# omnirevolve/omnirevolve-image-processor

Hardware: AMD Instinct MI355X
Metric: Mpx/s end-to-end (color->order) (higher is better)
Workload: dtype u8/i32 raster + f32/f64 geometry; 1 GPU; 4096x4096 BGR image, 8 colour layers, stages 02->12 (k-means fit, masks, edges, contours, scale, sort, intra dedup, cross dedup, plot order), default A4 canvas 8400x11880; parallelism=one GPU, one pipeline per colour layer, ops_last_step_rank0=4261, exchange=none

## Files before the change

omnirevolve-image-processor_amd/csrc/raster04.hip:

```cpp
#include "bitplane.h"
#include "walker.h"
#include <rocprim/rocprim.hpp>
#include <algorithm>
#include <cstdlib>

__global__ __launch_bounds__(256) void k_gather_head_layers(const unsigned* __restrict__ keys, const unsigned* __restrict__ cs, unsigned nc, unsigned* __restrict__ out) {
    unsigned i = blockIdx.x * 256 + threadIdx.x;
    if (i < nc) out[i] = keys[cs[i]] >> 26;
}

__global__ __launch_bounds__(64) void k_trace(WalkArgs A) {
    unsigned i = blockIdx.x;
    if (i >= A.nc) return;
    trace_component(A, A.comp_order ? A.comp_order[i] : i);
}
__global__ __launch_bounds__(64) void k_write_walks(WalkArgs A, int layer, const unsigned* __restrict__ kept_slots, const unsigned long long* __restrict__ kept_off, unsigned n_kept,
                                                    unsigned long long total, unsigned chunk) {
    for (unsigned long long ci = blockIdx.x; ci * chunk < total; ci += gridDim.x) {
        const unsigned long long p0 = ci * chunk, p1 = p0 + chunk < total ? p0 + chunk : total;
        write_chunk(A, layer, kept_slots, kept_off, n_kept, p0, p1);
    }
}
__global__ void k_totals_flag(const int* __restrict__ over, unsigned* __restrict__ pad_of_total) { *pad_of_total = (unsigned)*over; }
struct WSum {
// ... 337 lines not shown
    layer_first[K] = NC;
    for (int l = 0; l < K; l++) A.total_fg[l] = (long long)R.h_cs[layer_first[l + 1]] - (long long)R.h_cs[layer_first[l]];
    {
        unsigned long long *kin, *kout; unsigned *idin, *idout;
        { Carve L; L.each(NC, kin, kout, idin, idout); HIPC(c, L.commit(LN(c).vtmp[VT0_ORDER_SORT], 64)); }
        hipLaunchKernelGGL(k_comp_order_keys, dim3(cdiv(NC, 256)), block, 0, LN(c).stream, keys, comp_start, NC, kin, idin);
        HIPC(c, orip_with_tmp(c, [&](void* tmp, size_t& bytes) { return rocprim::radix_sort_pairs(tmp, bytes, kin, kout, idin, idout, (size_t)NC, 0, 40, LN(c).stream); }));
        R.order = LN(c).vtmp[VT0_ORDER].as<unsigned>();
        HIPC(c, hipMemcpyAsync(LN(c).vtmp[VT0_ORDER].p, idout, (size_t)NC * 4, hipMemcpyDeviceToDevice, LN(c).stream));
    }
    HIPC(c, LN(c).vtmp[VT0_WINFO].ensure((size_t)2 * M * sizeof(WalkInfo) + 64));
    A.memo = LN(c).vtmp[VT0_MEMO].as<unsigned>(); A.winfo = LN(c).vtmp[VT0_WINFO].as<WalkInfo>();
    HIPC(c, LN(c).vtmp[VT0_LOG_USED].ensure((size_t)(NC + 1) * 4 + 64));
    A.log_used = LN(c).vtmp[VT0_LOG_USED].as<unsigned>();
    HIPC(c, hipStreamSynchronize(LN(c).stream));
    R.ready = true;
    if (!getenv("ORIP_TRACE_LATE"))
        for (int l = 0; l < R.K; l++) {
            if (R.layer_first[l] == R.layer_first[l + 1]) continue;
            LaneGuard g(c, l + 1);
            if (!g.ok) continue;
            HIPC(c, orip_pf08_drain(c));
            ORIP_TRY(trace_launch(c, R, l, trace_log_f0()));
        }
    return 0;
}

static int trace_launch(orip_ctx* c, Prep04& R, int layer, unsigned F) {
    const unsigned c0 = R.layer_first[layer], c1 = R.layer_first[layer + 1];
    const unsigned b0 = R.h_cs[c0], b1 = R.h_cs[c1];
    const unsigned Ml = b1 - b0, NCl = c1 - c0;
    const size_t plane = (size_t)R.A.plane;
    if ((uint64_t)F * R.M + (uint64_t)256 * R.NC + 64 >= 0xffffffffull) ORIP_FAIL(c, "skeleton too large for the walk logs (factor %u)", F);
    const size_t nlog = (size_t)F * Ml + (size_t)64 * NCl + 8, nstep = (size_t)F * Ml + (size_t)256 * NCl + 8;
    WalkStore& WS = c->wstore[layer];
    WS.epoch++; WS.n = 0;
    HIPC(c, WS.log.ensure(nlog * 16 + 64));
    HIPC(c, LN(c).vtmp[VTL_STEPLOG].ensure(nstep + 64));
    WalkArgs A = R.A;
    A.logbuf = WS.log.as<unsigned>() - 4 * ((size_t)F * b0 + (size_t)64 * c0);
    A.steplog = LN(c).vtmp[VTL_STEPLOG].as<u8>() - ((size_t)F * b0 + (size_t)256 * c0);
    A.cap_factor = F; A.comp_order = R.order + c0; A.nc = NCl;
    int* d_over = &LN(c).flags.as<LaneFlags>()->trace_overflow; A.overflow = d_over;
    if (R.chains) HIPC(c, hipStreamWaitEvent(LN(c).stream, c->ln[0].ev3, 0));
    if (R.F[layer])
        hipLaunchKernelGGL(k_clear_visited_layer, dim3(cdiv(Ml, 256)), dim3(256), 0, LN(c).stream, A.st + plane * layer, A.lin + b0, (int64_t)Ml);
    hipLaunchKernelGGL(k_clear_memo_layer, dim3(cdiv((int64_t)2 * Ml, 256)), dim3(256), 0, LN(c).stream, reinterpret_cast<uint4*>(A.memo + plane * 8 * layer), A.lin + b0, (int64_t)2 * Ml);
    HIPC(c, hipMemsetAsync(A.winfo + 2 * (size_t)b0, 0, (size_t)2 * Ml * sizeof(WalkInfo), LN(c).stream));
    HIPC(c, hipMemsetAsync(d_over, 0, 4, LN(c).stream));
    if (getenv("ORIP_WALK_DBG")) {
        HIPC(c, LN(c).vtmp[VT_LEAVES].ensure((size_t)NCl * 256 + 64)); HIPC(c, hipMemsetAsync(LN(c).vtmp[VT_LEAVES].p, 0, (size_t)NCl * 256, LN(c).stream));
        A.dbg = LN(c).vtmp[VT_LEAVES].as<unsigned long long>() - 32ull * c0;
    }
    { ProfScope ps(c, "k_trace"); hipLaunchKernelGGL(k_trace, dim3(NCl), dim3(64), 0, LN(c).stream, A); }
    HIPC(c, hipGetLastError());
    R.F[layer] = F; R.launched[layer] = true;
    return 0;
}
static int trace_finish(orip_ctx* c, Prep04& R, int layer) {
    const unsigned c0 = R.layer_first[layer], c1 = R.layer_first[layer + 1];
    const unsigned b0 = R.h_cs[c0], b1 = R.h_cs[c1];
    const unsigned Ml = b1 - b0;
    dim3 block(256);
    int* d_over = &LN(c).flags.as<LaneFlags>()->trace_overflow;
    const unsigned nslots = 2u * Ml, sl0 = 2u * b0;
    const size_t ns1 = (size_t)nslots + 1;
    WSum *ws, *wo; { Carve L; L.each(ns1, ws, wo); HIPC(c, L.commit(LN(c).vtmp[VTL_CAPS], 256)); }
    WalkStore& WS = c->wstore[layer];
    WSum h_tot; unsigned log_shift = 0; WalkArgs A;
    for (;;) {
    log_shift = (unsigned)((size_t)R.F[layer] * b0 + (size_t)64 * c0);
    A = R.A;
    A.logbuf = WS.log.as<unsigned>() - 4 * (size_t)log_shift;
    A.steplog = LN(c).vtmp[VTL_STEPLOG].as<u8>() - ((size_t)R.F[layer] * b0 + (size_t)256 * c0);
    A.cap_factor = R.F[layer]; A.overflow = d_over;
    hipLaunchKernelGGL(k_winfo_lens, dim3(cdiv(nslots + 1, 256)), block, 0, LN(c).stream, A, sl0, nslots, ws);
    { WSum zero; zero.pts = 0; zero.paths = zero.own = zero.pieces = zero.pad = 0; HIPC(c, orip_with_tmp(c, [&](void* tmp, size_t& bytes) { return rocprim::exclusive_scan(tmp, bytes, ws, wo, zero, ns1, rocprim::plus<WSum>(), LN(c).stream); })); }
    hipLaunchKernelGGL(k_totals_flag, dim3(1), dim3(1), 0, LN(c).stream, d_over, &wo[nslots].pad);
    HIPC(c, hipMemcpyAsync(&h_tot, wo + nslots, sizeof(WSum), hipMemcpyDeviceToHost, LN(c).stream));
    {
        const unsigned NCl = c1 - c0;
        WS.ent_cap = (int64_t)8 * Ml + 64;
        HIPC(c, WS.lxy.ensure(((size_t)R.F[layer] * Ml + (size_t)64 * NCl + 8) * 8 + 64));
        HIPC(c, WS.ent_idx.ensure((size_t)WS.ent_cap * 4 + 64));
        HIPC(c, WS.cnt.ensure(64));
        HIPC(c, hipMemsetAsync(WS.cnt.p, 0, 4, LN(c).stream));
        hipLaunchKernelGGL(k_ent_fill, dim3(NCl, 8), block, 0, LN(c).stream, A, c0, log_shift, WS.lxy.as<int2>(), WS.ent_idx.as<unsigned>(), WS.cnt.as<unsigned>(), (unsigned)WS.ent_cap);
    }
    HIPC(c, hipStreamSynchronize(LN(c).stream));
    if (!h_tot.pad) break;
    if (h_tot.pad == 2) ORIP_FAIL(c, "internal error: the walker of layer %d stopped making progress", layer);
    ORIP_TRY(trace_launch(c, R, layer, R.F[layer] * 4));
    }
    if (getenv("ORIP_WALK_DBG")) {
        const unsigned NCl = c1 - c0;
        std::vector<unsigned long long> h((size_t)NCl * 32);
        HIPC(c, hipMemcpy(h.data(), LN(c).vtmp[VT_LEAVES].p, h.size() * 8, hipMemcpyDeviceToHost));
        unsigned long long tot[32] = {0}; size_t big = 0;
        for (size_t i = 0; i < h.size(); i++) tot[i % 32] += h[i];
        for (size_t i = 0; i < NCl; i++) if (h[i * 32 + 7] > h[big * 32 + 7]) big = i;
        const unsigned long long* d = &h[big * 32];
        fprintf(stderr, "[walk dbg] layer %d NC=%u M=%u F=%u: w1=%llu s1=%llu w2=%llu s2=%llu hit=%llu det=%llu tiles=%llu | largest fg=%llu: w1=%llu s1=%llu w2=%llu s2=%llu hit=%llu det=%llu tiles=%llu jumped=%llu calls=%llu rounds=%llu\n",
                layer, NCl, Ml, R.F[layer], tot[0], tot[1], tot[2], tot[3], tot[4], tot[5], tot[6], d[7], d[0], d[1], d[2], d[3], d[4], d[5], d[6], d[15], d[22], d[23]);
        if (d[8]) fprintf(stderr, "[walk prof] layer %d largest component: cycles total=%llu window loads=%llu scans=%llu look-ups=%llu | look-ups=%llu loop exits=%llu\n",
                          layer, d[8], d[9], d[10], d[11], d[12], d[13]);
        if (d[8]) fprintf(stderr, "[walk prof]   inside the look-ups: duplicate check %llu cycles (exact check in %llu look-ups); forced stretches %llu cycles in %llu calls, %llu rounds; stepping loop %llu cycles; walk start + end %llu cycles\n", d[14], d[20], d[16], d[17], d[18], d[19], d[21]);
    }
    const unsigned long long h_pts = h_tot.pts; const unsigned h_paths = h_tot.paths, h_own = h_tot.own, h_pieces = h_tot.pieces;
    DPolys& P = c->polys[ORIP_SLOT_CONTOURS][layer];
    P.total = (int64_t)h_pts; P.n = (int64_t)h_paths;
    P.virt = true; P.pts_ok = false; P.vident = true; P.vlayer = layer; P.vepoch = WS.epoch; P.scaled = false;
    HIPC(c, P.off.ensure((size_t)(P.n + 1) * 8 + 64));
    HIPC(c, WS.walk.ensure((size_t)std::max(h_paths, 1u) * sizeof(VWalk) + 64));
    HIPC(c, WS.piece.ensure((size_t)std::max(h_pieces, 1u) * sizeof(VPiece) + 64));
    HIPC(c, WS.own.ensure((size_t)std::max(h_own, 1u) * 8 + 64));
    HIPC(c, LN(c).vtmp[VTL_CELLS].ensure((size_t)std::max(h_paths, 1u) * 4 + 64));
    unsigned* kept_slots = LN(c).vtmp[VTL_CELLS].as<unsigned>();
    WS.n = P.n; WS.W = R.A.W; WS.n_own = h_own;
    hipLaunchKernelGGL(k_vwalk_fill, dim3(cdiv(nslots + 1, 256)), block, 0, LN(c).stream, A, sl0, nslots, wo, log_shift,
                       WS.walk.as<VWalk>(), WS.piece.as<VPiece>(), kept_slots, P.off.as<int64_t>());
    if (h_paths) {
        ProfScope ps(c, "k_write_walks");
        const unsigned chunk = 2048;
        hipLaunchKernelGGL(k_vown, dim3((unsigned)std::min<unsigned long long>(((unsigned long long)h_own + chunk - 1) / chunk, 262144ull)), dim3(64), 0, LN(c).stream, A, kept_slots, WS.walk.as<VWalk>(), h_paths,
                           WS.own.as<int2>(), h_own, chunk);
    }
    HIPC(c, hipGetLastError());
    R.launched[layer] = false;
    return 0;
}

int orip_contours_layer_impl(orip_ctx* c, int layer, bool sync) {
    Prep04* R = static_cast<Prep04*>(c->prep04);
    if (!R || !R->ready) ORIP_FAIL(c, "orip_contours_prepare has not run");
    if (layer < 0 || layer >= R->K) ORIP_FAIL(c, "bad layer %d (prepared for %d layers)", layer, R->K);
    if (R->M == 0 || R->layer_first[layer] == R->layer_first[layer + 1]) return 0;
    ORIP_LANE(c, layer + 1);
    if (!R->launched[layer]) ORIP_TRY(trace_launch(c, *R, layer, trace_log_f0()));
    ORIP_TRY(trace_finish(c, *R, layer));
    if (sync) HIPC(c, hipStreamSynchronize(LN(c).stream));
    return 0;
}
extern "C" int orip_contours_layer(orip_ctx* c, int layer) {
    orip_enter(c);
    return orip_contours_layer_impl(c, layer, true);
}

extern "C" int orip_find_contours(orip_ctx* c) {
    orip_enter(c);
    ORIP_TRY(orip_contours_prepare(c));
    Prep04& R = *static_cast<Prep04*>(c->prep04);
    if (R.M == 0) return 0;
    for (int l = 0; l < R.K; l++) if (R.layer_first[l] != R.layer_first[l + 1] && !R.launched[l]) { ORIP_LANE(c, l + 1); ORIP_TRY(trace_launch(c, R, l, trace_log_f0())); }
    for (int l = 0; l < R.K; l++) if (R.launched[l]) { ORIP_LANE(c, l + 1); ORIP_TRY(trace_finish(c, R, l)); HIPC(c, hipStreamSynchronize(LN(c).stream)); }
    return 0;
}
// ... 10 lines not shown
```

omnirevolve-image-processor_amd/csrc/walker.h:

```cpp
#pragma once
#include <cstdint>
#include "../../include/orip.h"
#if defined(__HIPCC__)
#define ORIP_HD __host__ __device__
#else
#define ORIP_HD
struct int2 { int x, y; };
static inline int2 make_int2(int x, int y) { return int2{x, y}; }
#endif
typedef uint8_t u8;
#define ST_FG 0x80
#define ST_VIS 0x40
#define ST_JUN 2
#define ST_END 1
#define ST_DEG2 0x04
#define ST_CHAIN 0x08
#define ST_CHAIN_END 0x10
#define ORIP_CHAIN_SENTINEL 0xffffffffu
#ifndef ORIP_CHAIN_MIN
#define ORIP_CHAIN_MIN 24
#endif

struct WalkInfo {
    unsigned len_kept;
    unsigned n_own;
    unsigned step_begin;
    unsigned log_i1;
    unsigned R;
    unsigned flags;
};

struct WalkArgs {
    int H, W; int64_t plane;
    u8* st;
    const unsigned* keys; const unsigned* lin; const unsigned* comp_start; unsigned nc;
    long long total_fg[ORIP_MAX_LAYERS];
    const unsigned* comp_order;
    unsigned* memo;
    unsigned* logbuf;
    u8* steplog;
    unsigned cap_factor;
    WalkInfo* winfo;
    int* overflow;
    unsigned* log_used;
    const unsigned* cref;
    const unsigned* cpix;
    const unsigned long long* pts_off; const unsigned* path_off;
    unsigned long long layer_pts_base[ORIP_MAX_LAYERS]; unsigned layer_path_base[ORIP_MAX_LAYERS];
    int32_t* pts[ORIP_MAX_LAYERS]; int64_t* off[ORIP_MAX_LAYERS];
    unsigned long long* dbg;
};

#ifndef ORIP_WALK_LEAD
#define ORIP_WALK_LEAD 16
#endif
#ifndef ORIP_WALK_BATCH
#define ORIP_WALK_BATCH 16u
#endif
namespace walk_detail {
#if defined(__HIP_DEVICE_COMPILE__) && defined(ORIP_WALK_PROF)
#define WPROF_NOW() ((unsigned long long)__builtin_amdgcn_s_memtime())
#else
#define WPROF_NOW() 0ull
#endif
#define WPROF_ADD(acc, t0) do { (acc) += WPROF_NOW() - (t0); } while (0)

enum { EV_DEAD = 1,
       EV_PEND = 2,
       EV_LIMIT = 3,
       EV_HOME = 4,
       EV_BATCH = 5 };
struct Hot { unsigned steps, limit, nb, nbatch, allow; };

#if defined(__HIP_DEVICE_COMPILE__)
#define WT 64
#define WTP (WT + 4)
#define WB_FG ST_FG
#define WB_VIS ST_VIS
#define WB_RING 0x20
#define WB_HOME 0x10
#define WB_JUN ST_JUN
#define WB_END ST_END
struct Wave {
    int lane;
    u8* tile;
    unsigned lds_base;
    int tx0, ty0; bool have; unsigned nload;
    unsigned pl;
    int li;
    bool reload;
    int lastk;
    int noff, noffa, dplv;
    unsigned sel;
    int thr;
    int va, v;
    int rec;
    unsigned home;
    unsigned codes_done, marks_done;
    u8* st; int W, H;
    unsigned long long t_tile = 0;
    mutable unsigned long long n_exact = 0;
    u8* dtab;
    __device__ Wave() : lane((int)(threadIdx.x & 63)), tx0(0), ty0(0), have(false), nload(0), pl(0), li(0), reload(true), lastk(8), noff(0), noffa(0), dplv(0), sel(0), thr(-64),
                        va(0), v(0), rec(0), home(~0u), codes_done(0), marks_done(0), st(nullptr), W(0), H(0) {
        __shared__ u8 lds_tile[WT * WTP];
        __shared__ u8 lds_dup[8192];
        tile = lds_tile; lds_base = (unsigned)(uintptr_t)lds_tile; dtab = lds_dup;
    }
    __device__ void init(u8* st_, int W_, int H_) {
        st = st_; W = W_; H = H_;
        if (lane < 8) {
            const int dx = (int)((0x9224u >> (2 * lane)) & 3u) - 1, dy = (int)((0xA940u >> (2 * lane)) & 3u) - 1;
            noff = dy * WTP + dx; dplv = dy * W + dx; sel = (unsigned)WB_VIS << lane;
        }
        if (lane == 8) thr = -48;
        noffa = noff + (int)lds_base;
    }
    __device__ bool leader() const { return lane == 0; }
    __device__ unsigned l0() const { return (unsigned)lane; }
    __device__ unsigned nl() const { return 64u; }
    __device__ void fence() const { __builtin_amdgcn_fence(__ATOMIC_SEQ_CST, "wavefront"); __builtin_amdgcn_s_waitcnt(0); }
    __device__ unsigned ld0(const unsigned* p) const { unsigned x = 0; if (lane == 0) x = *p; return (unsigned)__builtin_amdgcn_readfirstlane((int)x); }
    __device__ void ld0_rec(const unsigned* p, unsigned& cont, unsigned& en, unsigned& begin) const {
        uint4 x = make_uint4(0, 0, 0, 0); if (lane == 0) x = *reinterpret_cast<const uint4*>(p);
        cont = (unsigned)__builtin_amdgcn_readfirstlane((int)x.y); en = (unsigned)__builtin_amdgcn_readfirstlane((int)x.z); begin = (unsigned)__builtin_amdgcn_readfirstlane((int)x.w);
    }
    __device__ u8 ld_state(unsigned lin) const { return __hip_atomic_load(st + lin, __ATOMIC_RELAXED, __HIP_MEMORY_SCOPE_AGENT); }
    __device__ void or_visited(unsigned lin) const {
        const uintptr_t a = (uintptr_t)(st + lin);
        atomicOr(reinterpret_cast<unsigned*>(a & ~(uintptr_t)3), (unsigned)ST_VIS << (8u * (unsigned)(a & 3)));
    }
    __device__ unsigned my_step(unsigned steps) const { return steps - 1u - ((steps - 1u - (unsigned)lane) & 63u); }
    __device__ void flush_marks(unsigned steps) {
        if (steps > marks_done) {
            const unsigned t = my_step(steps);
            if (t < steps && t >= marks_done && (rec & 2)) or_visited((unsigned)rec >> 5);
            marks_done = steps;
        }
    }
    __device__ void sync_marks(unsigned steps) { flush_marks(steps); fence(); }
    __device__ void begin_walk(unsigned home_) { codes_done = 0; marks_done = 0; home = home_; }
    __device__ void flush_codes(u8* slog, unsigned room, unsigned steps) {
        if (steps > codes_done) {
            const unsigned t = my_step(steps);
            if (t < steps && t >= codes_done && t < room) slog[t] = (u8)(((unsigned)rec >> 2) & 7u);
            codes_done = steps;
        }
        flush_marks(steps);
    }
    __device__ unsigned pending(unsigned first) const { return (unsigned)__shfl(rec, (int)((first + (unsigned)lane) & 63u), 64) >> 2; }
    __device__ void load_tile(int cx, int cy, unsigned steps) {
        const unsigned long long t_0 = WPROF_NOW();
        flush_marks(steps);
        fence();
        const int lead_x = lastk < 8 ? ((int)((0x9224u >> (2 * lastk)) & 3u) - 1) * ORIP_WALK_LEAD : 0;
        const int lead_y = lastk < 8 ? ((int)((0xA940u >> (2 * lastk)) & 3u) - 1) * ORIP_WALK_LEAD : 0;
        tx0 = ((cx - (WT / 2 - 8) + lead_x) >> 4) << 4; ty0 = cy - WT / 2 + lead_y;
        const int y = ty0 + lane;
        u8* row = tile + lane * WTP;
        const uint32_t ring_row = (lane == 0 || lane == WT - 1) ? 0x20202020u : 0u;
        if (y < 0 || y >= H) { for (int j = 0; j < WT; j += 4) *reinterpret_cast<uint32_t*>(row + j) = 0x20202020u; }
        else if ((W & 15) == 0 && tx0 >= 0 && tx0 + WT <= W && (tx0 & 15) == 0 && ((uintptr_t)st & 15) == 0) {
            typedef unsigned v4u __attribute__((ext_vector_type(4)));
            const v4u* src = reinterpret_cast<const v4u*>(st + (size_t)y * W + tx0);
            v4u q[4];
#pragma unroll
            for (int j = 0; j < 4; j++) q[j] = __builtin_nontemporal_load(src + j);
#pragma unroll
            for (int j = 0; j < 4; j++) {
                uint32_t w4[4] = {q[j].x | ring_row, q[j].y | ring_row, q[j].z | ring_row, q[j].w | ring_row};
                if (j == 0) w4[0] |= 0x20u;
                if (j == 3) w4[3] |= 0x20000000u;
#pragma unroll
                for (int t = 0; t < 4; t++) *reinterpret_cast<uint32_t*>(row + 16 * j + 4 * t) = w4[t];
            }
        } else if ((W & 3) == 0 && tx0 >= 0 && tx0 + WT <= W && ((uintptr_t)st & 3) == 0) {
            const uint32_t* src = reinterpret_cast<const uint32_t*>(st + (size_t)y * W + tx0);
            uint32_t w[WT / 4];
#pragma unroll
            for (int j = 0; j < WT / 4; j++) w[j] = __hip_atomic_load(src + j, __ATOMIC_RELAXED, __HIP_MEMORY_SCOPE_AGENT);
#pragma unroll
            for (int j = 0; j < WT / 4; j++) {
                uint32_t x = w[j] | ring_row;
                if (j == 0) x |= 0x20u;
                if (j == WT / 4 - 1) x |= 0x20000000u;
                *reinterpret_cast<uint32_t*>(row + 4 * j) = x;
            }
        } else {
            for (int j = 0; j < WT; j++) {
                int x = tx0 + j; u8 bte = (x >= 0 && x < W) ? ld_state((unsigned)((size_t)y * W + x)) : (u8)0;
                if (ring_row || j == 0 || j == WT - 1) bte |= WB_RING;
                row[j] = bte;
            }
        }
        have = true; nload++;
        __builtin_amdgcn_fence(__ATOMIC_SEQ_CST, "wavefront");
        if (home != ~0u && steps > 0 && lane == 0) {
            const int hx = (int)(home % (unsigned)W) - tx0, hy = (int)(home / (unsigned)W) - ty0;
            if ((unsigned)hx < (unsigned)WT && (unsigned)hy < (unsigned)WT) tile[hy * WTP + hx] |= WB_HOME;
        }
        __builtin_amdgcn_fence(__ATOMIC_SEQ_CST, "wavefront");
        WPROF_ADD(t_tile, t_0);
    }
    __device__ void set_cursor(unsigned lin) { pl = lin; reload = true; lastk = 8; }
    __device__ void place(unsigned steps) {
        const int px = (int)(pl % (unsigned)W), py = (int)(pl / (unsigned)W);
        int lx = px - tx0, ly = py - ty0;
        if (!have || (unsigned)(lx - 1) > (unsigned)(WT - 3) || (unsigned)(ly - 1) > (unsigned)(WT - 3)) { load_tile(px, py, steps); lx = px - tx0; ly = py - ty0; }
        li = ly * WTP + lx; reload = false;
    }
    __device__ void mark_cursor(u8 gv) {
        if (lane == 0) {
            st[pl] = (u8)(gv | ST_VIS);
            if (have) {
                const int lx = (int)(pl % (unsigned)W) - tx0, ly = (int)(pl / (unsigned)W) - ty0;
                if ((unsigned)lx < (unsigned)WT && (unsigned)ly < (unsigned)WT) tile[ly * WTP + lx] |= WB_VIS;
            }
        }
        fence();
    }
    __device__ void flag_home() {
        if (lane == 0 && home != ~0u) {
            const int hx = (int)(home % (unsigned)W) - tx0, hy = (int)(home / (unsigned)W) - ty0;
            if (have && (unsigned)hx < (unsigned)WT && (unsigned)hy < (unsigned)WT) tile[hy * WTP + hx] |= WB_HOME;
        }
        fence();
    }
    __device__ void probe(unsigned allow, unsigned steps, unsigned& m_any, unsigned& m_unvis) {
        if (reload) place(steps);
        va = li + noff;
        v = (int)(signed char)tile[va];
        const unsigned m_fg = (unsigned)__builtin_amdgcn_ballot_w64(v < 0), m_un = (unsigned)__builtin_amdgcn_ballot_w64(v < -64);
        m_any = m_fg & allow & 0xffu;
        m_unvis = m_any & m_un;
    }
    __device__ u8 step(int k, bool fresh, unsigned steps) {
        const int vk = __builtin_amdgcn_readlane(v, k);
        li += __builtin_amdgcn_readlane(noff, k);
        pl = (unsigned)((int)pl + __builtin_amdgcn_readlane(dplv, k));
        lastk = k;
        const int r = (int)((((pl << 3) | (unsigned)k) << 2) | (fresh ? 2u : 0u));
        rec = lane == (int)(steps & 63u) ? r : rec;
        if (fresh) tile[va] = (u8)(v | (int)((sel >> k) & WB_VIS));
        reload = (vk & WB_RING) != 0;
        return (u8)((vk & (ST_FG | ST_VIS | ST_END | ST_JUN)) | (fresh ? ST_VIS : 0));
    }
    __device__ int resume_flagged(unsigned steps) {
        const u8 cell = tile[li];
        if (cell & WB_HOME) {
            if (pl == home) return 2;
            if (cell & ST_CHAIN) return 3;
            if (lane == 0) tile[li] = (u8)(cell & ~WB_HOME);
            fence();
            if (!(cell & WB_RING)) return 1;
        }
        if (cell & WB_RING) { reload = true; place(steps); return 1; }
        return 0;
    }
    __device__ bool came_along_chain() const {
        if (reload || lastk >= 8) return false;
        const u8 cell = tile[li];
        if (cell & WB_RING) return false;
        const u8 nbv = lane < 8 ? tile[li + noff] : (u8)0;
        const unsigned chain_nb = (unsigned)__ballot((nbv & ST_FG) && (nbv & ST_CHAIN)) & 0xffu;
        const unsigned back = 0x80u >> lastk;
        return (chain_nb & back) != 0u && (chain_nb & ~back) == 0u;
    }
    __device__ void unflag_cursor(unsigned steps) {
        if (reload) place(steps);
        const u8 cell = tile[li];
        if (lane == 0) tile[li] = (u8)(cell & ~WB_HOME);
        fence();
// ... 93 lines not shown
        "v_readlane_b32 %[tmp], %[dplv], %[k]\n\t"                                                                    \
        "s_and_b32 %[fr2], %[frmask], 2\n\t"                                                                          \
        "s_add_i32 %[pl], %[pl], %[tmp]\n\t"                                                                          \
        "s_lshl3_add_u32 %[r], %[pl], %[k]\n\t"                                                                       \
        "s_lshl2_add_u32 %[r], %[r], %[fr2]\n\t"                                                                      \
        "v_writelane_b32 %[rec], %[r], m0\n\t"                                                                        \
        "s_add_i32 %[nb], %[nb], 1\n\t"                                                                               \
        "s_andn2_b32 %[nb], %[nb], %[frmask]\n\t"                                                                     \
        "s_lshr_b32 %[tmp], 0x80, %[k]\n\t"                                                                           \
        "s_andn2_b32 %[allow], 0xff, %[tmp]\n\t"                                                                      \
        "s_add_i32 %[steps], %[steps], 1\n\t"                                                                         \
        "s_add_i32 m0, m0, 1\n\t"                                                                                     \
        "s_cmp_ge_u32 %[steps], %[limit]\n\t"                                                                         \
        "s_cbranch_scc1 L_limit%=\n\t"                                                                                \
        "s_cmp_ge_u32 %[nb], %[nbatch]\n\t"                                                                           \
        "s_cbranch_scc1 L_batch%=\n\t"
        asm volatile(
            "s_mov_b32 %[m0save], m0\n\t"
            "s_and_b32 m0, %[steps], 63\n\t"
            "v_add_u32 %[va], %[li], %[noffa]\n\t"
            "ds_read_i8 %[v], %[va]\n\t"
            ORIP_WALK_HALF("A", "va", "v", "vb", "w")
            ORIP_WALK_HALF("B", "vb", "w", "va", "v")
            "s_branch L_A%=\n\t"
            "L_batch%=:\n\t"
            "s_mov_b32 %[ev], 5\n\t"
            "s_branch L_out%=\n\t"
            "L_dead%=:\n\t"
            "s_mov_b32 %[ev], 1\n\t"
            "s_branch L_out%=\n\t"
            "L_pend%=:\n\t"
            "s_mov_b32 %[ev], 2\n\t"
            "s_branch L_out%=\n\t"
            "L_limit%=:\n\t"
            "s_mov_b32 %[ev], 3\n\t"
            "L_out%=:\n\t"
            "s_waitcnt lgkmcnt(0)\n\t"
            "s_mov_b32 m0, %[m0save]\n\t"
            : [ev] "=&s"(ev), [li] "+s"(s_li), [pl] "+s"(s_pl), [allow] "+s"(s_allow), [steps] "+s"(s_steps), [nb] "+s"(s_nb),
              [rec] "+v"(rec), [va] "=&v"(r_va), [v] "=&v"(r_v), [vb] "=&v"(r_vb), [w] "=&v"(r_w), [t2] "=&v"(r_t2),
              [m_any] "=&s"(m_any), [m_un] "=&s"(m_un), [m] "=&s"(m), [frmask] "=&s"(frmask), [fr2] "=&s"(fr2), [fr40] "=&s"(fr40), [r] "=&s"(r), [tmp] "=&s"(tmp),
              [k] "=&s"(k), [m0save] "=&s"(m0save)
            : [limit] "s"(s_limit), [nbatch] "s"(s_nbatch), [noff] "v"(noff), [noffa] "v"(noffa), [dplv] "v"(dplv), [sel] "v"(sel), [thr] "v"(thr)
            : "vcc", "scc", "memory");
#undef ORIP_WALK_HALF
        li = s_li; pl = s_pl; h.allow = s_allow; h.steps = s_steps; h.nb = s_nb;
        const unsigned back = ~s_allow & 0xffu;
        lastk = back ? 7 - (int)__builtin_ctz(back) : 8;
        return ev;
    }
};
#else
struct Wave {
    u8 nv[8]; unsigned nload = 0; unsigned long long t_tile = 0, n_exact = 0;
    unsigned pl = 0, home = ~0u;
    unsigned pend_state = 0;
    u8* st = nullptr; int W = 0, H = 0;
    void init(u8* st_, int W_, int H_) { st = st_; W = W_; H = H_; }
    bool leader() const { return true; }
    unsigned l0() const { return 0u; }
    unsigned nl() const { return 1u; }
    void fence() const {}
    unsigned ld0(const unsigned* p) const { return *p; }
    void ld0_rec(const unsigned* p, unsigned& cont, unsigned& en, unsigned& begin) const { cont = p[1]; en = p[2]; begin = p[3]; }
    u8 ld_state(unsigned lin) const { return st[lin]; }
    void set_cursor(unsigned lin) { pl = lin; }
    void mark_cursor(u8 v) { st[pl] = (u8)(v | ST_VIS); }
    void flag_home() {}
    void sync_marks(unsigned) {}
    void begin_walk(unsigned home_) { home = home_; }
    void flush_codes(u8*, unsigned, unsigned) {}
    unsigned pending(unsigned) const { return pend_state; }
    int resume_flagged(unsigned) { return 0; }
    void log_code(u8* slog, unsigned room, unsigned idx, int k) { if (idx < room) slog[idx] = (u8)k; }
    void probe(unsigned allow, unsigned, unsigned& m_any, unsigned& m_unvis) {
        const int dxs[8] = {-1, 0, 1, -1, 1, -1, 0, 1}, dys[8] = {-1, -1, -1, 0, 0, 1, 1, 1};
        const int px = (int)(pl % (unsigned)W), py = (int)(pl / (unsigned)W);
        m_any = m_unvis = 0;
        for (int k = 0; k < 8; k++) {
            int xx = px + dxs[k], yy = py + dys[k]; nv[k] = 0;
            if (xx < 0 || xx >= W || yy < 0 || yy >= H) continue;
            u8 v = st[(size_t)yy * W + xx]; nv[k] = v;
            if ((v & ST_FG) && ((allow >> k) & 1u)) { m_any |= 1u << k; if (!(v & ST_VIS)) m_unvis |= 1u << k; }
        }
    }
    u8 step(int k, bool mark, unsigned) {
        const int dxs[8] = {-1, 0, 1, -1, 1, -1, 0, 1}, dys[8] = {-1, -1, -1, 0, 0, 1, 1, 1};
        pl = (unsigned)((int)pl + dys[k] * W + dxs[k]);
        if (mark) st[pl] = (u8)(nv[k] | ST_VIS);
        return (u8)(nv[k] | (mark ? ST_VIS : 0));
    }
    int run(Hot& h, u8* slog, unsigned room) {
        while (true) {
            unsigned m_any, m_un;
            probe(h.allow, h.steps, m_any, m_un);
            const bool fresh = m_un != 0;
            const unsigned m = fresh ? m_un : m_any;
            if (!m) return EV_DEAD;
            if (fresh && h.nb) return EV_PEND;
            const int k = __builtin_ctz(m);
            log_code(slog, room, h.steps, k);
            step(k, fresh, h.steps);
            h.steps++;
            h.allow = 0xffu & ~(0x80u >> k);
            if (!fresh) { pend_state = (pl << 3) | (unsigned)k; h.nb++; }
            if (pl == home) return EV_HOME;
            if (h.steps >= h.limit) return EV_LIMIT;
            if (h.nb >= h.nbatch) return EV_BATCH;
        }
    }
    unsigned bcast(unsigned v, int) const { return v; }
    int first(bool pred) const { return pred ? 0 : -1; }
    unsigned dup_distance(unsigned, unsigned) const { return 0u; }
    unsigned scan_lin = 0; u8 scan_st = 0;
    unsigned scan(const unsigned* lin, unsigned q0, unsigned e, u8 need) {
        for (unsigned q = q0; q < e; q++) { u8 v = st[lin[q]]; if (((v & need) == need) && !(v & ST_VIS)) { scan_lin = lin[q]; scan_st = v; return q; } }
        return e;
    }
    void scan2(int dx, int dy, int& ox, int& oy, int& tx, int& ty) const { ox = dx; oy = dy; tx = dx; ty = dy; }
};
#endif
ORIP_HD inline int ffs8(unsigned m) { return __builtin_ctz(m); }
ORIP_HD inline int nbx(int k) { return (int)((0x9224u >> (2 * k)) & 3u) - 1; }
ORIP_HD inline int nby(int k) { return (int)((0xA940u >> (2 * k)) & 3u) - 1; }
}

struct PlainReader {
    ORIP_HD void ld0_rec(const unsigned* p, unsigned& cont, unsigned& en, unsigned& begin) const { cont = p[1]; en = p[2]; begin = p[3]; }
};

template <class WaveT>
ORIP_HD inline unsigned long long log_resolve(const unsigned* logbuf, const WaveT& wv, unsigned rec, unsigned long long f) {
    while (true) {
        unsigned cont, en, begin; wv.ld0_rec(&logbuf[4ull * rec], cont, en, begin);
        if (f < en) return f;
        if (cont >= begin) return (unsigned long long)cont + (f - en) % (unsigned long long)(en - cont);
        f = (unsigned long long)cont + (f - en); rec = cont;
    }
}

ORIP_HD inline bool close_to(int W, unsigned a, unsigned b) {
    const int ddx = (int)(a % (unsigned)W) - (int)(b % (unsigned)W), ddy = (int)(a / (unsigned)W) - (int)(b / (unsigned)W);
    return ddx * ddx + ddy * ddy < 3;
}

template <class WaveT>
ORIP_HD inline void walk_close_tail(const WalkArgs& A, const WaveT& wv, unsigned slot, WalkInfo& wi) {
    if (!(wi.flags & 2u)) return;
    unsigned lo = 0, hi = A.nc;
    while (lo < hi) { unsigned mid = (lo + hi) >> 1; if (2u * A.comp_start[mid + 1] <= slot) lo = mid + 1; else hi = mid; }
    const unsigned b = A.comp_start[lo], fg = A.comp_start[lo + 1] - b, rel = slot - 2u * b;
    const unsigned s = A.lin[b + (rel >= fg ? rel - fg : rel)];
    const unsigned i = wi.log_i1 - 1;
    const unsigned long long f = log_resolve(A.logbuf, wv, i, (unsigned long long)i + wi.R);
    const unsigned endp = A.logbuf[4ull * f] >> 3;
    wi.flags = 0;
    if (close_to(A.W, s, endp)) { wi.flags = 1; wi.len_kept++; }
}

ORIP_HD inline void trace_component(const WalkArgs& A, unsigned c) {
    using namespace walk_detail;
    Wave wv;
    const unsigned b = A.comp_start[c], e = A.comp_start[c + 1], fg = e - b;
    const int layer = (int)(A.keys[b] >> 26);
    u8* st = A.st + A.plane * layer;
    unsigned* memo = A.memo + (size_t)A.plane * layer * 8;
    const int W = A.W, H = A.H;
    wv.init(st, W, H);
    const long long total_fg = A.total_fg[layer];
    const unsigned F = A.cap_factor;
    const unsigned log_base = F * b + 64u * c, log_cap = F * fg + 64u;
    const unsigned step_base = F * b + 256u * c, step_cap = F * fg + 256u;
    unsigned logcur = 0, stepcur = 0;
    bool over = false, stalled = false;
    unsigned long long d_w1 = 0, d_s1 = 0, d_w2 = 0, d_s2 = 0, d_hit = 0, d_det = 0, d_jump = 0;
    unsigned long long t_scan = 0, t_flush = 0, n_flush = 0, n_ev = 0, t_f3 = 0, t_chain = 0, n_chain = 0, n_round = 0, t_run = 0, t_walk = 0; const unsigned long long t_begin = WPROF_NOW();
    auto finish = [&](unsigned slot, unsigned long long len, unsigned n_own, unsigned sbeg, unsigned log_i1, unsigned R, unsigned flags) {
        if (wv.leader()) { WalkInfo wi; wi.len_kept = len >= 5 ? (unsigned)len : 0u; wi.n_own = n_own; wi.step_begin = sbeg; wi.log_i1 = log_i1; wi.R = R; wi.flags = flags; A.winfo[slot] = wi; }
    };
    auto tscan = [&](unsigned q0, u8 need) { const unsigned long long t_0 = WPROF_NOW(); const unsigned r = wv.scan(A.lin, q0, e, need); WPROF_ADD(t_scan, t_0); return r; };
    const unsigned long long g1 = (unsigned long long)(total_fg * 2);
    for (unsigned q = tscan(b, ST_FG | ST_END); q < e; q = tscan(q + 1, ST_FG | ST_END)) {
        unsigned s = wv.scan_lin;
        wv.set_cursor(s);
        const unsigned sbeg = step_base + stepcur;
        u8* slog = A.steplog + (size_t)sbeg; const unsigned room = step_cap - stepcur;
        wv.begin_walk(~0u);
        wv.mark_cursor(ST_FG | ST_END);
        unsigned steps = 0, allow = 0xffu; d_w1++;
        while (true) {
            unsigned m_any, m_unvis;
            wv.probe(allow, steps, m_any, m_unvis);
            if (!m_unvis) break;
            const int k = ffs8(m_unvis);
            if (steps >= room) over = true;
            wv.log_code(slog, room, steps, k);
            const u8 v = wv.step(k, true, steps);
            steps++;
            if ((steps & 63u) == 0) wv.flush_codes(slog, room, steps);
            allow = 0xffu & ~(0x80u >> k);
            if (v & (ST_JUN | ST_END)) break;
            if ((unsigned long long)steps > g1) break;
        }
        stepcur += steps; d_s1 += steps;
        wv.flush_codes(slog, room, steps);
        wv.sync_marks(steps);
        finish(2u * b + (q - b), 1ull + steps, steps, sbeg, 0u, 0u, 0u);
    }
    const unsigned g2 = fg * 4u;
    const unsigned nbatch0 = wv.nl() < ORIP_WALK_BATCH ? wv.nl() : ORIP_WALK_BATCH;
    for (unsigned q = tscan(b, ST_FG); q < e && !over && !stalled; q = tscan(q + 1, ST_FG)) {
        const unsigned long long t_w0 = WPROF_NOW();
        unsigned s = wv.scan_lin;
        wv.set_cursor(s);
        const unsigned sbeg = step_base + stepcur;
        u8* slog = A.steplog + (size_t)sbeg; const unsigned room = step_cap - stepcur;
        wv.begin_walk(s);
        wv.mark_cursor(wv.scan_st);
        d_w2++;
        Hot h; h.steps = 0;
        h.limit = 0; h.nb = 0;
        h.nbatch = nbatch0;
        h.allow = 0xffu;
        unsigned long long tail_len = 0; unsigned tail_i1 = 0, tail_R = 0;
        unsigned nofresh = 0;
        unsigned flush_mark = 0;
        unsigned drop = 0;
        auto discard_run = [&]() {
            if (nofresh) {
                const unsigned run_begin = log_base + logcur;
                for (unsigned t = wv.l0(); t < nofresh; t += wv.nl()) memo[A.logbuf[4ull * (run_begin + t)]] = 0u;
                wv.fence();
                nofresh = 0;
            }
        };
        auto flush_ = [&](bool ext, unsigned ext_state) -> int {
            const unsigned nb = h.nb - drop;
            if (!nb) { h.nb = 0; return 0; }
            const unsigned steps_b = h.steps - h.nb;
            if (steps_b > flush_mark) { discard_run(); h.nbatch = nbatch0; }
            const unsigned myS = ext ? ext_state : wv.pending(steps_b);
            const unsigned run_begin = log_base + logcur;
            const unsigned me = wv.l0();
            const bool act = me < nb;
            wv.fence();
            unsigned mi = 0;
            if (act) mi = memo[myS];
            const unsigned long long t_c = WPROF_NOW();
            const unsigned dist = wv.dup_distance(act ? myS + 1u : 0u, nb);
            const bool dup = act && dist != 0; const unsigned dsrc = me - dist;
            t_f3 += WPROF_NOW() - t_c;
            const bool hit_old = act && mi != 0;
            const int js = wv.first(hit_old || dup);
            const unsigned ncommit = js < 0 ? nb : (unsigned)js;
            if (logcur + nofresh + ncommit > log_cap) { over = true; h.nb = 0; return 2; }
            if (me < ncommit) { const unsigned idx = run_begin + nofresh + me; A.logbuf[4ull * idx] = myS; memo[myS] = idx + 1; }
            if (js < 0) { nofresh += nb; h.nb = 0; flush_mark = h.steps; return 0; }
            const unsigned ev_mi = wv.bcast(dup ? run_begin + nofresh + dsrc + 1u : mi, js);
            nofresh += (unsigned)js;
            h.steps = steps_b + (unsigned)js + 1;
            const unsigned i = ev_mi - 1;
            const unsigned long long R = (unsigned long long)g2 + 1ull - h.steps;
            if (i < run_begin) d_hit++; else d_det++;
            if (nofresh) {
                const unsigned end = run_begin + nofresh;
                for (unsigned t = me; t < nofresh; t += wv.nl()) { unsigned* p = A.logbuf + 4ull * (run_begin + t); p[1] = i; p[2] = end; p[3] = run_begin; }
                logcur += nofresh;
                nofresh = 0;
            }
            tail_i1 = ev_mi; tail_R = (unsigned)R; tail_len = R;
            h.nb = 0;
            return 1;
        };
        auto flush = [&]() -> int { const unsigned long long t_0 = WPROF_NOW(); n_flush++; const int r = flush_(false, 0u); WPROF_ADD(t_flush, t_0); return r; };
        int ended = 0;
        unsigned stall = 0, stall_steps = ~0u;
#if defined(__HIP_DEVICE_COMPILE__)
        unsigned last_jump_end = ~0u;
        auto chain_jump = [&]() -> int {
            if (!A.cref || wv.pl == last_jump_end || wv.lastk >= 8 || wv.came_along_chain()) { wv.unflag_cursor(h.steps); return 0; }
            const unsigned lane = wv.l0();
            wv.flush_codes(slog, room, h.steps);
            wv.fence();
            int res = 0; bool moved = false;
            unsigned idx = wv.ld0(A.cref + (size_t)A.plane * layer + wv.pl);
            unsigned q_up = A.cpix[idx + lane + 1u], q_dn = A.cpix[idx - lane - 1u];
            const unsigned prev_px = (unsigned)((int)wv.pl - (nby(wv.lastk) * W + nbx(wv.lastk)));
            const unsigned c_m = wv.bcast(q_dn, 0), c_p = wv.bcast(q_up, 0);
            int dir;
            if (c_p == prev_px) dir = -1; else if (c_m == prev_px) dir = 1;
            else dir = c_m == ORIP_CHAIN_SENTINEL ? 1 : -1;
            bool first_round = true;
            while (true) {
                const long long room_left = (long long)(room < g2 ? room : g2) - 80ll - (long long)h.steps;
                if (room_left < 8) break;
                const unsigned q = first_round ? (dir > 0 ? q_up : q_dn) : A.cpix[(unsigned)((int)idx + dir * (int)(lane + 1u))];
                first_round = false;
                const int sent = wv.first(q == ORIP_CHAIN_SENTINEL);
                const bool valid = sent < 0 || (int)lane < sent;
                u8 sb = 0; if (valid) sb = wv.ld_state(q);
                const bool fr = !(sb & ST_VIS);
                const bool fr0 = wv.bcast(fr ? 1u : 0u, 0) != 0u;
                const bool stop = !valid || fr != fr0 || q == wv.home;
                int r = wv.first(stop); if (r < 0) r = 64;
                bool go_on = r == 64 || wv.bcast((valid && q != wv.home) ? 1u : 0u, r < 64 ? r : 0) != 0u;
                if ((long long)r > room_left) { r = (int)room_left; go_on = false; }
                if (r < (moved ? 1 : 8)) break;
                unsigned qp = (unsigned)__shfl_up((int)q, 1, 64); if (lane == 0) qp = wv.pl;
                const int dd = (int)q - (int)qp; const int dy = W > 2 ? (dd > 1 ? 1 : (dd < -1 ? -1 : 0)) : (int)(q >> (W - 1)) - (int)(qp >> (W - 1)); const int dx = dd - dy * W;
                const int kk = (dy + 1) * 3 + (dx + 1); const int k = kk > 4 ? kk - 1 : kk;
                const unsigned myst = (q << 3) | (unsigned)k;
                const unsigned nbp = h.nb;
                if (!fr0 && nbp + (unsigned)r <= wv.nl()) {
                    const unsigned pend = nbp ? wv.pending(h.steps - nbp) : 0u;
                    const unsigned ext = (unsigned)__shfl((int)myst, (int)((lane - nbp) & 63u), 64);
                    if ((int)lane < r && h.steps + lane < room) slog[h.steps + lane] = (u8)k;
                    moved = true;
                    h.steps += (unsigned)r; h.nb = nbp + (unsigned)r;
                    n_flush++;
                    res = flush_(true, lane < nbp ? pend : ext);
                    if (res) break;
                } else {
                    if (nbp) { res = flush(); if (res) break; }
                    if ((int)lane < r && h.steps + lane < room) slog[h.steps + lane] = (u8)k;
                    moved = true;
                    if (fr0) {
                        if ((int)lane < r) wv.or_visited(q);
                        h.steps += (unsigned)r;
                    } else {
                        h.steps += (unsigned)r; h.nb = (unsigned)r;
                        n_flush++;
                        res = flush_(true, myst);
                        if (res) break;
                    }
                }
                d_jump += (unsigned)r; n_round++;
                wv.pl = wv.bcast(q, r - 1); wv.lastk = (int)wv.bcast((unsigned)k, r - 1); h.allow = 0xffu & ~(0x80u >> wv.lastk);
                idx = (unsigned)((int)idx + dir * r);
                if (!go_on) break;
            }
            if (moved) {
                wv.codes_done = h.steps; wv.marks_done = h.steps; last_jump_end = wv.pl;
                if (!res) { wv.have = false; wv.reload = true; wv.place(h.steps); }
            } else if (!res) wv.unflag_cursor(h.steps);
            return res;
        };
#endif
        WPROF_ADD(t_walk, t_w0);
        while (true) {
            if (h.steps >= room) { over = true; break; }
            unsigned lim = (h.steps & ~63u) + 64u;
            if (lim > g2 + 1u) lim = g2 + 1u;
            if (lim > room) lim = room;
            h.limit = lim;
            const unsigned long long t_r0 = WPROF_NOW();
            int ev = wv.run(h, slog, room);
            WPROF_ADD(t_run, t_r0);
            n_ev++;
            if (ev == EV_DEAD) {
                int f = wv.resume_flagged(h.steps);
#if defined(__HIP_DEVICE_COMPILE__)
                if (f == 3) { const unsigned long long t_0 = WPROF_NOW(); n_chain++; ended = chain_jump(); WPROF_ADD(t_chain, t_0); if (ended) break; f = 1; }
#endif
                if (f == 1) {
                    if (h.steps == stall_steps && ++stall > 8u) { stalled = true; break; }
                    if (h.steps != stall_steps) { stall_steps = h.steps; stall = 0; }
                    continue;
                }
                if (f == 0) break;
                ev = EV_HOME;
            }
            if (ev == EV_HOME) { drop = h.nb ? 1u : 0u; break; }
            if (ev == EV_PEND) { ended = flush(); if (ended) break; continue; }
            if (ev == EV_LIMIT) {
                if ((h.steps & 63u) == 0) wv.flush_codes(slog, room, h.steps);
                if (h.steps > g2) { drop = h.nb ? 1u : 0u; break; }
                if (h.nb < h.nbatch) continue;
            }
            ended = flush(); if (ended) break;
            h.nbatch = h.nbatch * 2u < wv.nl() ? h.nbatch * 2u : wv.nl();
        }
        const unsigned long long t_w1 = WPROF_NOW();
        if (!ended && h.nb > drop) ended = flush();
        wv.flush_codes(slog, room, h.steps);
        if (ended != 1) discard_run();
        wv.sync_marks(h.steps);
        if (ended == 2) break;
        const unsigned steps = h.steps;
        stepcur += steps; d_s2 += steps;
        unsigned long long len = 1ull + steps + tail_len;
        unsigned flags = 0;
        if (ended == 1) flags = 2;
        else if (len >= 2 && close_to(W, s, wv.pl)) { flags = 1; len++; }
        finish(2u * b + fg + (q - b), len >= 2 ? len : 0, steps, sbeg, tail_i1, tail_R, flags);
        WPROF_ADD(t_walk, t_w1);
    }
    if (A.log_used && wv.leader()) A.log_used[c] = logcur;
    if (over && wv.leader()) *A.overflow = 1;
    if (stalled && wv.leader()) *A.overflow = 2;
    if (A.dbg && wv.leader()) {
        unsigned long long* d = A.dbg + 32ull * c; d[0] = d_w1; d[1] = d_s1; d[2] = d_w2; d[3] = d_s2; d[4] = d_hit; d[5] = d_det; d[6] = wv.nload; d[7] = (unsigned long long)fg;
        d[8] = WPROF_NOW() - t_begin; d[9] = wv.t_tile; d[10] = t_scan; d[11] = t_flush; d[12] = n_flush; d[13] = n_ev; d[14] = t_f3; d[15] = d_jump; d[16] = t_chain; d[17] = n_chain; d[18] = n_round; d[19] = t_run; d[20] = wv.n_exact; d[21] = t_walk;
        d[22] = n_chain; d[23] = n_round;
    }
}

ORIP_HD inline void write_chunk(const WalkArgs& A, int layer, const unsigned* kept, const unsigned long long* kept_off, unsigned n_kept, unsigned long long p0, unsigned long long p1) {
    using namespace walk_detail;
    Wave wv;
    const int W = A.W;
    int2* outp = reinterpret_cast<int2*>(A.pts[layer]);
    unsigned lo = 0, hi = n_kept;
    while (hi - lo > 1) { const unsigned mid = (lo + hi) >> 1; if (kept_off[mid] <= p0) lo = mid; else hi = mid; }
    for (unsigned i = lo; i < n_kept; i++) {
        const unsigned slot = kept[i];
        const unsigned long long ws = kept_off[i];
        if (ws >= p1) break;
        const WalkInfo wi = A.winfo[slot];
        const unsigned long long L = wi.len_kept;
        const unsigned long long ta = (p0 > ws ? p0 : ws) - ws, tb = (p1 < ws + L ? p1 : ws + L) - ws;
        if (ta >= tb) continue;
        int2* out = outp + ws;
        unsigned clo = 0, chi = A.nc;
        while (clo < chi) { unsigned mid = (clo + chi) >> 1; if (2u * A.comp_start[mid + 1] <= slot) clo = mid + 1; else chi = mid; }
        const unsigned b = A.comp_start[clo], fg = A.comp_start[clo + 1] - b, rel = slot - 2u * b;
        const unsigned s = A.lin[b + (rel >= fg ? rel - fg : rel)];
        const int x0 = (int)(s % (unsigned)W), y0 = (int)(s / (unsigned)W);
        if (wv.leader()) {
            if (ta == 0) { out[0] = make_int2(x0, y0); A.off[layer][i + 1] = (int64_t)(ws + L); }
            if ((wi.flags & 1u) && tb == L) out[L - 1] = make_int2(x0, y0);
        }
        const unsigned long long own_a = ta > 1 ? ta : 1, own_b = tb < (unsigned long long)wi.n_own + 1 ? tb : (unsigned long long)wi.n_own + 1;
        if (own_a < own_b) {
            int cx = x0, cy = y0;
            for (unsigned long long c0 = 0; c0 < own_a - 1; c0 += wv.nl()) {
                const unsigned long long t = c0 + wv.l0();
                int dx = 0, dy = 0;
                if (t < own_a - 1) { const int k = A.steplog[(size_t)wi.step_begin + t]; dx = nbx(k); dy = nby(k); }
                int ox, oy, tx, ty; wv.scan2(dx, dy, ox, oy, tx, ty);
                cx += tx; cy += ty;
            }
            for (unsigned long long t0 = own_a; t0 < own_b; t0 += wv.nl()) {
                const unsigned long long t = t0 + wv.l0();
                int dx = 0, dy = 0;
                if (t < own_b) { const int k = A.steplog[(size_t)wi.step_begin + t - 1]; dx = nbx(k); dy = nby(k); }
                int ox, oy, tx, ty; wv.scan2(dx, dy, ox, oy, tx, ty);
                if (t < own_b) out[t] = make_int2(cx + ox, cy + oy);
                cx += tx; cy += ty;
            }
        }
        if (wi.log_i1) {
            const unsigned long long tail0 = (unsigned long long)wi.n_own + 1;
            unsigned long long ua = (ta > tail0 ? ta : tail0) - tail0, ub = (tb < tail0 + wi.R ? tb : tail0 + wi.R);
            if (ub > tail0 && ua < ub - tail0) {
                ub -= tail0;
                int2* o2 = out + tail0;
// ... 90 lines not shown
```

Baseline: 305.7 Mpx/s.

## Skip redundant mark flushes and device fences in the contour walker tile loads

```diff
diff --git a/omnirevolve-image-processor_amd/csrc/raster04.hip b/omnirevolve-image-processor_amd/csrc/raster04.hip
--- a/omnirevolve-image-processor_amd/csrc/raster04.hip
+++ b/omnirevolve-image-processor_amd/csrc/raster04.hip
@@ -413,6 +413,7 @@
         HIPC(c, LN(c).vtmp[VT_LEAVES].ensure((size_t)NCl * 256 + 64)); HIPC(c, hipMemsetAsync(LN(c).vtmp[VT_LEAVES].p, 0, (size_t)NCl * 256, LN(c).stream));
         A.dbg = LN(c).vtmp[VT_LEAVES].as<unsigned long long>() - 32ull * c0;
     }
+    A.old_waits = getenv("ORIP_WALK_OLD_WAITS") ? 1u : 0u;
     { ProfScope ps(c, "k_trace"); hipLaunchKernelGGL(k_trace, dim3(NCl), dim3(64), 0, LN(c).stream, A); }
     HIPC(c, hipGetLastError());
     R.F[layer] = F; R.launched[layer] = true;
@@ -461,8 +462,8 @@
         for (size_t i = 0; i < h.size(); i++) tot[i % 32] += h[i];
         for (size_t i = 0; i < NCl; i++) if (h[i * 32 + 7] > h[big * 32 + 7]) big = i;
         const unsigned long long* d = &h[big * 32];
-        fprintf(stderr, "[walk dbg] layer %d NC=%u M=%u F=%u: w1=%llu s1=%llu w2=%llu s2=%llu hit=%llu det=%llu tiles=%llu | largest fg=%llu: w1=%llu s1=%llu w2=%llu s2=%llu hit=%llu det=%llu tiles=%llu jumped=%llu calls=%llu rounds=%llu\n",
-                layer, NCl, Ml, R.F[layer], tot[0], tot[1], tot[2], tot[3], tot[4], tot[5], tot[6], d[7], d[0], d[1], d[2], d[3], d[4], d[5], d[6], d[15], d[22], d[23]);
+        fprintf(stderr, "[walk dbg] layer %d NC=%u M=%u F=%u: w1=%llu s1=%llu w2=%llu s2=%llu hit=%llu det=%llu tiles=%llu | largest fg=%llu: w1=%llu s1=%llu w2=%llu s2=%llu hit=%llu det=%llu tiles=%llu jumped=%llu calls=%llu rounds=%llu nowait=%llu early=%llu entered=%llu starts=%llu first=%llu\n",
+                layer, NCl, Ml, R.F[layer], tot[0], tot[1], tot[2], tot[3], tot[4], tot[5], tot[6], d[7], d[0], d[1], d[2], d[3], d[4], d[5], d[6], d[15], d[22], d[23], d[25], d[26], d[27], d[28], d[29]);
         if (d[8]) fprintf(stderr, "[walk prof] layer %d largest component: cycles total=%llu window loads=%llu scans=%llu look-ups=%llu | look-ups=%llu loop exits=%llu\n",
                           layer, d[8], d[9], d[10], d[11], d[12], d[13]);
         if (d[8]) fprintf(stderr, "[walk prof]   inside the look-ups: duplicate check %llu cycles (exact check in %llu look-ups); forced stretches %llu cycles in %llu calls, %llu rounds; stepping loop %llu cycles; walk start + end %llu cycles\n", d[14], d[20], d[16], d[17], d[18], d[19], d[21]);
diff --git a/omnirevolve-image-processor_amd/csrc/walker.h b/omnirevolve-image-processor_amd/csrc/walker.h
--- a/omnirevolve-image-processor_amd/csrc/walker.h
+++ b/omnirevolve-image-processor_amd/csrc/walker.h
@@ -49,6 +49,7 @@
     unsigned long long layer_pts_base[ORIP_MAX_LAYERS]; unsigned layer_path_base[ORIP_MAX_LAYERS];
     int32_t* pts[ORIP_MAX_LAYERS]; int64_t* off[ORIP_MAX_LAYERS];
     unsigned long long* dbg;
+    unsigned old_waits;
 };
 
 #ifndef ORIP_WALK_LEAD
@@ -97,6 +98,10 @@
     int rec;
     unsigned home;
     unsigned codes_done, marks_done;
+    unsigned start = ~0u; int start_x = 0, start_y = 0;
+    bool old_waits = false;
+    bool skip_wait = false;
+    unsigned long long n_nowait = 0, n_early = 0, n_starts = 0, n_first = 0;
     u8* st; int W, H;
     unsigned long long t_tile = 0;
     mutable unsigned long long n_exact = 0;
@@ -139,7 +144,10 @@
         }
     }
     __device__ void sync_marks(unsigned steps) { flush_marks(steps); fence(); }
-    __device__ void begin_walk(unsigned home_) { codes_done = 0; marks_done = 0; home = home_; }
+    __device__ void begin_walk(unsigned home_, unsigned start_) {
+        codes_done = 0; marks_done = 0; home = home_;
+        start = start_; start_x = (int)(start_ % (unsigned)W); start_y = (int)(start_ / (unsigned)W);
+    }
     __device__ void flush_codes(u8* slog, unsigned room, unsigned steps) {
         if (steps > codes_done) {
             const unsigned t = my_step(steps);
@@ -151,8 +159,10 @@
     __device__ unsigned pending(unsigned first) const { return (unsigned)__shfl(rec, (int)((first + (unsigned)lane) & 63u), 64) >> 2; }
     __device__ void load_tile(int cx, int cy, unsigned steps) {
         const unsigned long long t_0 = WPROF_NOW();
-        flush_marks(steps);
-        fence();
+        if (old_waits || !(skip_wait || steps == 0u)) { flush_marks(steps); fence(); }
+        else if (skip_wait) n_nowait++;
+        else n_first++;
+        skip_wait = false;
         const int lead_x = lastk < 8 ? ((int)((0x9224u >> (2 * lastk)) & 3u) - 1) * ORIP_WALK_LEAD : 0;
         const int lead_y = lastk < 8 ? ((int)((0xA940u >> (2 * lastk)) & 3u) - 1) * ORIP_WALK_LEAD : 0;
         tx0 = ((cx - (WT / 2 - 8) + lead_x) >> 4) << 4; ty0 = cy - WT / 2 + lead_y;
@@ -195,10 +205,16 @@
         }
         have = true; nload++;
         __builtin_amdgcn_fence(__ATOMIC_SEQ_CST, "wavefront");
-        if (home != ~0u && steps > 0 && lane == 0) {
-            const int hx = (int)(home % (unsigned)W) - tx0, hy = (int)(home / (unsigned)W) - ty0;
-            if ((unsigned)hx < (unsigned)WT && (unsigned)hy < (unsigned)WT) tile[hy * WTP + hx] |= WB_HOME;
-        }
+        if (start != ~0u && lane == 0) {
+            const int hx = start_x - tx0, hy = start_y - ty0;
+            if ((unsigned)hx < (unsigned)WT && (unsigned)hy < (unsigned)WT) {
+                u8 f = 0;
+                if (!old_waits) f |= WB_VIS;
+                if (home != ~0u && steps > 0) f |= WB_HOME;
+                tile[hy * WTP + hx] |= f;
+            }
+        }
+        if (!old_waits && start != ~0u && (unsigned)(start_x - tx0) < (unsigned)WT && (unsigned)(start_y - ty0) < (unsigned)WT) n_starts++;
         __builtin_amdgcn_fence(__ATOMIC_SEQ_CST, "wavefront");
         WPROF_ADD(t_tile, t_0);
     }
@@ -213,11 +229,11 @@
         if (lane == 0) {
             st[pl] = (u8)(gv | ST_VIS);
             if (have) {
-                const int lx = (int)(pl % (unsigned)W) - tx0, ly = (int)(pl / (unsigned)W) - ty0;
+                const int lx = start_x - tx0, ly = start_y - ty0;
                 if ((unsigned)lx < (unsigned)WT && (unsigned)ly < (unsigned)WT) tile[ly * WTP + lx] |= WB_VIS;
             }
         }
-        fence();
+        if (old_waits) fence(); else __builtin_amdgcn_fence(__ATOMIC_SEQ_CST, "wavefront");
     }
     __device__ void flag_home() {
         if (lane == 0 && home != ~0u) {
@@ -417,7 +433,8 @@
 };
 #else
 struct Wave {
-    u8 nv[8]; unsigned nload = 0; unsigned long long t_tile = 0, n_exact = 0;
+    u8 nv[8]; unsigned nload = 0; unsigned long long t_tile = 0, n_exact = 0, n_nowait = 0, n_early = 0, n_starts = 0, n_first = 0;
+    bool old_waits = false;
     unsigned pl = 0, home = ~0u;
     unsigned pend_state = 0;
     u8* st = nullptr; int W = 0, H = 0;
@@ -433,7 +450,7 @@
     void mark_cursor(u8 v) { st[pl] = (u8)(v | ST_VIS); }
     void flag_home() {}
     void sync_marks(unsigned) {}
-    void begin_walk(unsigned home_) { home = home_; }
+    void begin_walk(unsigned home_, unsigned) { home = home_; }
     void flush_codes(u8*, unsigned, unsigned) {}
     unsigned pending(unsigned) const { return pend_state; }
     int resume_flagged(unsigned) { return 0; }
@@ -532,13 +549,14 @@
     unsigned* memo = A.memo + (size_t)A.plane * layer * 8;
     const int W = A.W, H = A.H;
     wv.init(st, W, H);
+    wv.old_waits = A.old_waits != 0u;
     const long long total_fg = A.total_fg[layer];
     const unsigned F = A.cap_factor;
     const unsigned log_base = F * b + 64u * c, log_cap = F * fg + 64u;
     const unsigned step_base = F * b + 256u * c, step_cap = F * fg + 256u;
     unsigned logcur = 0, stepcur = 0;
     bool over = false, stalled = false;
-    unsigned long long d_w1 = 0, d_s1 = 0, d_w2 = 0, d_s2 = 0, d_hit = 0, d_det = 0, d_jump = 0;
+    unsigned long long d_w1 = 0, d_s1 = 0, d_w2 = 0, d_s2 = 0, d_hit = 0, d_det = 0, d_jump = 0, n_entered = 0;
     unsigned long long t_scan = 0, t_flush = 0, n_flush = 0, n_ev = 0, t_f3 = 0, t_chain = 0, n_chain = 0, n_round = 0, t_run = 0, t_walk = 0; const unsigned long long t_begin = WPROF_NOW();
     auto finish = [&](unsigned slot, unsigned long long len, unsigned n_own, unsigned sbeg, unsigned log_i1, unsigned R, unsigned flags) {
         if (wv.leader()) { WalkInfo wi; wi.len_kept = len >= 5 ? (unsigned)len : 0u; wi.n_own = n_own; wi.step_begin = sbeg; wi.log_i1 = log_i1; wi.R = R; wi.flags = flags; A.winfo[slot] = wi; }
@@ -550,7 +568,7 @@
         wv.set_cursor(s);
         const unsigned sbeg = step_base + stepcur;
         u8* slog = A.steplog + (size_t)sbeg; const unsigned room = step_cap - stepcur;
-        wv.begin_walk(~0u);
+        wv.begin_walk(~0u, s);
         wv.mark_cursor(ST_FG | ST_END);
         unsigned steps = 0, allow = 0xffu; d_w1++;
         while (true) {
@@ -580,7 +598,7 @@
         wv.set_cursor(s);
         const unsigned sbeg = step_base + stepcur;
         u8* slog = A.steplog + (size_t)sbeg; const unsigned room = step_cap - stepcur;
-        wv.begin_walk(s);
+        wv.begin_walk(s, s);
         wv.mark_cursor(wv.scan_st);
         d_w2++;
         Hot h; h.steps = 0;
@@ -645,10 +663,13 @@
         auto chain_jump = [&]() -> int {
             if (!A.cref || wv.pl == last_jump_end || wv.lastk >= 8 || wv.came_along_chain()) { wv.unflag_cursor(h.steps); return 0; }
             const unsigned lane = wv.l0();
+            unsigned idx_early = 0;
+            if (!wv.old_waits) { if (lane == 0) idx_early = A.cref[(size_t)A.plane * layer + wv.pl]; wv.n_early++; }
             wv.flush_codes(slog, room, h.steps);
             wv.fence();
-            int res = 0; bool moved = false;
-            unsigned idx = wv.ld0(A.cref + (size_t)A.plane * layer + wv.pl);
+            int res = 0; bool moved = false, marked = false;
+            unsigned idx = wv.old_waits ? wv.ld0(A.cref + (size_t)A.plane * layer + wv.pl) : (unsigned)__builtin_amdgcn_readfirstlane((int)idx_early);
+            n_entered++;
             unsigned q_up = A.cpix[idx + lane + 1u], q_dn = A.cpix[idx - lane - 1u];
             const unsigned prev_px = (unsigned)((int)wv.pl - (nby(wv.lastk) * W + nbx(wv.lastk)));
             const unsigned c_m = wv.bcast(q_dn, 0), c_p = wv.bcast(q_up, 0);
@@ -691,6 +712,7 @@
                     moved = true;
                     if (fr0) {
                         if ((int)lane < r) wv.or_visited(q);
+                        marked = true;
                         h.steps += (unsigned)r;
                     } else {
                         h.steps += (unsigned)r; h.nb = (unsigned)r;
@@ -706,7 +728,7 @@
             }
             if (moved) {
                 wv.codes_done = h.steps; wv.marks_done = h.steps; last_jump_end = wv.pl;
-                if (!res) { wv.have = false; wv.reload = true; wv.place(h.steps); }
+                if (!res) { wv.have = false; wv.reload = true; wv.skip_wait = !marked && !wv.old_waits; wv.place(h.steps); }
             } else if (!res) wv.unflag_cursor(h.steps);
             return res;
         };
@@ -767,6 +789,7 @@
         unsigned long long* d = A.dbg + 32ull * c; d[0] = d_w1; d[1] = d_s1; d[2] = d_w2; d[3] = d_s2; d[4] = d_hit; d[5] = d_det; d[6] = wv.nload; d[7] = (unsigned long long)fg;
         d[8] = WPROF_NOW() - t_begin; d[9] = wv.t_tile; d[10] = t_scan; d[11] = t_flush; d[12] = n_flush; d[13] = n_ev; d[14] = t_f3; d[15] = d_jump; d[16] = t_chain; d[17] = n_chain; d[18] = n_round; d[19] = t_run; d[20] = wv.n_exact; d[21] = t_walk;
         d[22] = n_chain; d[23] = n_round;
+        d[25] = wv.n_nowait; d[26] = wv.n_early; d[27] = n_entered; d[28] = wv.n_starts; d[29] = wv.n_first;
     }
 }
 
```

Result: no change. 305.5 Mpx/s (-0.1%).
